# GuidoManni/BodySLAM

Hardware: AMD Instinct MI355X
Metric: frames/sec depth+pose+back-proj, 640x480 seq (higher is better)
Workload: dtype f16

## Files before the change

### bodyslam_amd/_lib.py

```python
from __future__ import annotations

import ctypes as C
import os
from typing import Optional

import torch

_HERE = os.path.dirname(os.path.abspath(__file__))
LIB_PATH = os.environ.get("BODYSLAM_HIP_LIB") or os.path.join(_HERE, "libbodyslam_hip.so")

F32, F16, BF16 = 0, 1, 2
ACT_NONE, ACT_RELU, ACT_GELU, ACT_SOFTPLUS, ACT_SOFTPLUS_FAST = 0, 1, 2, 3, 4
OUT_PLAIN, OUT_SHUFFLE, OUT_QKV = 0, 1, 2

_TORCH2BS = {torch.float32: F32, torch.float16: F16, torch.bfloat16: BF16}
BS2TORCH = {F32: torch.float32, F16: torch.float16, BF16: torch.bfloat16}


class BodySlamHipError(RuntimeError):
    pass


class GemmDesc(C.Structure):
    _fields_ = [
# ... 71 lines not shown
    "bs_odo_p2p_step": [C.c_void_p, C.c_void_p, C.c_int32, C.c_int32, C.c_int32, C.c_void_p, C.c_void_p, C.c_int32, C.c_double, C.c_double, C.c_void_p,
                        C.c_void_p, C.c_void_p],
    "bs_tsdf_touch": [C.c_void_p, C.c_int32, C.c_int32, C.c_int32, C.c_void_p, C.c_void_p, C.c_double, C.c_double, C.c_void_p, C.c_void_p, C.c_void_p,
                      C.c_int32, C.c_int32, C.c_void_p, C.c_int32, C.c_void_p, C.c_void_p, C.c_void_p],
    "bs_tsdf_integrate": [C.c_void_p, C.c_void_p, C.c_int32, C.c_int32, C.c_void_p, C.c_void_p, C.c_void_p, C.c_void_p, C.c_int32, C.c_void_p, C.c_int32,
                          C.c_int32, C.c_double, C.c_double, C.c_void_p, C.c_void_p],
    "bs_tsdf_extract": [C.c_void_p, C.c_int32, C.c_void_p, C.c_void_p, C.c_int32, C.c_void_p, C.c_int32, C.c_int32, C.c_double, C.c_void_p, C.c_void_p,
                        C.c_void_p, C.c_void_p, C.c_void_p, C.c_void_p],
    "bs_tsdf_mesh": [C.c_void_p, C.c_int32, C.c_void_p, C.c_void_p, C.c_int32, C.c_void_p, C.c_int32, C.c_int32, C.c_double, C.c_void_p, C.c_int32] + [C.c_void_p] * 7,
    "bs_tsdf_raycast": [C.c_void_p, C.c_void_p, C.c_int32, C.c_int32, C.c_int32, C.c_double, C.c_double, C.c_void_p, C.c_void_p, C.c_int32, C.c_void_p,
                        C.c_int32, C.c_int32, C.c_double, C.c_double, C.c_void_p, C.c_void_p, C.c_void_p, C.c_void_p, C.c_void_p],
    "bs_attractor_step": [C.c_void_p] * 4 + [C.c_int32] * 8 + [C.c_void_p],
    "bs_add_resized": [C.c_void_p] * 3 + [C.c_int32] * 7 + [C.c_void_p],
    "bs_mlp2": [C.c_void_p, C.c_int32] + [C.c_void_p] * 5 + [C.c_int32] * 6 + [C.c_void_p],
    "bs_mlp2_add": [C.c_void_p] * 7 + [C.c_int32] * 10 + [C.c_void_p],
    "bs_projector_level": [C.c_void_p] * 10 + [C.c_int32] * 9 + [C.c_void_p],
    "bs_logbinom_depth": [C.c_void_p] * 8 + [C.c_int32] * 5 + [C.c_float, C.c_float, C.c_int32, C.c_void_p],
    "bs_logbinom_depth_ex": [C.c_void_p] * 7 + [C.c_int32] + [C.c_void_p] * 2 + [C.c_int32] * 5 + [C.c_float, C.c_float, C.c_int32, C.c_void_p],
    "bs_small_attention": [C.c_void_p, C.c_void_p, C.c_int32, C.c_int32, C.c_int32, C.c_int32, C.c_void_p],
    "bs_route_argmax": [C.c_void_p, C.c_int32, C.c_void_p, C.c_int32, C.c_void_p],
    "bs_postprocess_depth": [C.c_void_p] * 3 + [C.c_int32] * 6 + [C.c_void_p],
    "bs_cyclepose_im2col": [C.c_void_p] * 3 + [C.c_int32] * 4 + [C.c_void_p],
    "bs_cyclepose_im2col_window": [C.c_void_p] * 3 + [C.c_int32] * 8 + [C.c_void_p],
    "bs_instnorm_relu_nhwc": [C.c_void_p] * 4 + [C.c_int32] * 3 + [C.c_float, C.c_int32, C.c_void_p],
    "bs_avgpool_nhwc": [C.c_void_p, C.c_void_p, C.c_int32, C.c_int32, C.c_int32, C.c_void_p],
    "bs_cyclepose_head": [C.c_void_p] * 12 + [C.c_int32] * 3 + [C.c_void_p],
    "bs_backproject": [C.c_void_p, C.c_int32, C.c_int32, C.c_int32, C.c_void_p, C.c_double, C.c_double] + [C.c_void_p] * 6,
    "bs_pose_chain": [C.c_void_p, C.c_int32, C.c_void_p, C.c_void_p, C.c_void_p],
    "bs_pose_chain_from": [C.c_void_p, C.c_int32, C.c_void_p, C.c_void_p, C.c_void_p],
    "bs_pixel_to_3d": [C.c_void_p, C.c_int64, C.c_void_p, C.c_void_p, C.c_void_p],
# ... 426 lines not shown

def resize_bias_relu_nhwc(x, bias, out, B, Hin, Win, Cch, Hout, Wout, split=False):
    check(load_library().bs_resize_bias_relu_nhwc(p(x), p(bias), p(out), B, Hin, Win, Cch, Hout, Wout, 1 | (2 if split else 0), dt(out), stream_ptr()),
          "bs_resize_bias_relu_nhwc")


def attractor_step(A, bins_prev, bins_out, route, B, Hp, Wp, H, W, groups, n_bins, n_attr):
    check(load_library().bs_attractor_step(p(A), p(bins_prev), p(bins_out), p(route), B, Hp, Wp, H, W, groups, n_bins, n_attr,
                                           stream_ptr()), "bs_attractor_step")


def mlp2(x, ldx, W1, b1, W2, b2, out, M, K1, N1, N2, act2=ACT_SOFTPLUS_FAST):
    check(load_library().bs_mlp2(p(x), ldx, p(W1), p(b1), p(W2), p(b2), p(out), M, K1, N1, N2, act2, dt(x), stream_ptr()), "bs_mlp2")


def mlp2_add(emb, prev, W1, b1, W2, b2, out, B, Hp, Wp, H, W, K1, N1, N2, act2=ACT_SOFTPLUS_FAST, split=False):
    check(load_library().bs_mlp2_add(p(emb), p(prev), p(W1), p(b1), p(W2), p(b2), p(out), B, Hp, Wp, H, W, K1, N1, N2, act2,
                                     dt(emb) | (16 if split else 0), stream_ptr()), "bs_mlp2_add")


def projector_level(z, b_c1, emb_prev, Wc2, b_c2, We, b_e, x_out, emb_out, eh_out, B, Hl, Wl, H, W, PM, E, NE):
    check(load_library().bs_projector_level(p(z), p(b_c1), p(emb_prev), p(Wc2), p(b_c2), p(We), p(b_e), p(x_out), p(emb_out), p(eh_out), B, Hl, Wl,
                                            H, W, PM, E, NE, dt(z), stream_ptr()), "bs_projector_level")


def add_resized(x, prev, out, B, Hp, Wp, H, W, Cch, split=False):
    check(load_library().bs_add_resized(p(x), p(prev), p(out), B, Hp, Wp, H, W, Cch, dt(x) | (16 if split else 0), stream_ptr()),
          "bs_add_resized")


# ... 74 lines not shown
```

### bodyslam_amd/csrc/common.h

```cpp
#pragma once
#include <hip/hip_runtime.h>
#include <stdint.h>
#include <stdio.h>
#include <stdlib.h>

#include <atomic>

#include "../../include/bodyslam_hip.h"

namespace bs {

typedef _Float16 f16;
typedef __bf16 bf16;
typedef _Float16 f16x4 __attribute__((ext_vector_type(4)));
typedef _Float16 f16x8 __attribute__((ext_vector_type(8)));
typedef __bf16 bf16x4 __attribute__((ext_vector_type(4)));
typedef __bf16 bf16x8 __attribute__((ext_vector_type(8)));
typedef float f32x4 __attribute__((ext_vector_type(4)));
typedef float f32x16 __attribute__((ext_vector_type(16)));
typedef unsigned int u32x4 __attribute__((ext_vector_type(4)));
typedef unsigned int u32x2 __attribute__((ext_vector_type(2)));

void set_error(const char* fmt, ...);
const void* zero_page();
// ... 138 lines not shown

__device__ __forceinline__ int f8_pack4(float a, float b, float c, float d) {
    auto cl = [](float v) { return __builtin_amdgcn_fmed3f(v, -448.0f, 448.0f); };
    int r = 0;
    r = __builtin_amdgcn_cvt_pk_fp8_f32(cl(a), cl(b), r, false);
    r = __builtin_amdgcn_cvt_pk_fp8_f32(cl(c), cl(d), r, true);
    return r;
}
__device__ __forceinline__ void f8_unpack4(int packed, float (&o)[4]) {
    typedef float f32x2 __attribute__((ext_vector_type(2)));
    const f32x2 a = __builtin_amdgcn_cvt_pk_f32_fp8(packed, false), b = __builtin_amdgcn_cvt_pk_f32_fp8(packed, true);
    o[0] = a[0]; o[1] = a[1]; o[2] = b[0]; o[3] = b[1];
}
constexpr int F8_ACT_HI_EXP = BS_F8_ACT_HI_EXP, F8_ACT_LO_EXP = BS_F8_ACT_LO_EXP;

__device__ __forceinline__ void glds16(const void* gptr, void* lds_wave_base) {
    __builtin_amdgcn_global_load_lds((const __attribute__((address_space(1))) void*)gptr,
                                     (__attribute__((address_space(3))) void*)lds_wave_base, 16, 0, 0);
}

static inline int cdiv(int a, int b) { return (a + b - 1) / b; }
static inline int64_t cdiv64(int64_t a, int64_t b) { return (a + b - 1) / b; }

}
```

### bodyslam_amd/csrc/engine.hip

```cpp
#include <stdio.h>
#include <string.h>

#include <exception>
#include <map>
#include <string>
#include <tuple>
#include <type_traits>
#include <utility>
#include <memory>
#include <vector>

#include "common.h"

namespace {

constexpr char kMagic[8] = {'B', 'S', 'E', 'N', 'G', '0', '2', '\0'};
enum { KIND_WORKSPACE = 0, KIND_ZERO = 1, KIND_DATA = 2 };
enum { ARG_I64 = 0, ARG_F64 = 1, ARG_PTR = 2, ARG_NULL = 3, ARG_DESC = 4 };
enum { OP_CALL = 0, OP_SIGNAL = 1, OP_WAIT = 2 };

struct Arg {
    int64_t i = 0;
    double d = 0.0;
    void* p = nullptr;
// ... 28 lines not shown
}
#define BS_ENGINE_ENTRY(name) {#name, make_entry(name)}
const std::map<std::string, Entry>& entries() {
    static const std::map<std::string, Entry> m = {
        BS_ENGINE_ENTRY(bs_gemm),           BS_ENGINE_ENTRY(bs_attention),          BS_ENGINE_ENTRY(bs_attention_table),
        BS_ENGINE_ENTRY(bs_attention_table_corr),
        BS_ENGINE_ENTRY(bs_layernorm),      BS_ENGINE_ENTRY(bs_cast),               BS_ENGINE_ENTRY(bs_copy_f32),
        BS_ENGINE_ENTRY(bs_cast_split),     BS_ENGINE_ENTRY(bs_relu_split),         BS_ENGINE_ENTRY(bs_preprocess_patches),
        BS_ENGINE_ENTRY(bs_fill_rows),      BS_ENGINE_ENTRY(bs_upconv_tapsum),      BS_ENGINE_ENTRY(bs_small_attention),
        BS_ENGINE_ENTRY(bs_route_argmax),   BS_ENGINE_ENTRY(bs_resize_bilinear_nhwc), BS_ENGINE_ENTRY(bs_rank1_bias),
        BS_ENGINE_ENTRY(bs_postprocess_depth), BS_ENGINE_ENTRY(bs_logbinom_depth_ex), BS_ENGINE_ENTRY(bs_col_mean),
        BS_ENGINE_ENTRY(bs_attractor_step), BS_ENGINE_ENTRY(bs_add_resized),        BS_ENGINE_ENTRY(bs_instnorm_relu_nhwc),
        BS_ENGINE_ENTRY(bs_cyclepose_im2col), BS_ENGINE_ENTRY(bs_cyclepose_im2col_window), BS_ENGINE_ENTRY(bs_cyclepose_head),
        BS_ENGINE_ENTRY(bs_avgpool_nhwc),   BS_ENGINE_ENTRY(bs_mlp2),            BS_ENGINE_ENTRY(bs_mlp2_add),
        BS_ENGINE_ENTRY(bs_upconv_fused),   BS_ENGINE_ENTRY(bs_resize_bias_relu_nhwc), BS_ENGINE_ENTRY(bs_projector_level),
    };
    return m;
}

struct Op {
    int kind = OP_CALL, lane = 0;
    const Entry* entry = nullptr;
    std::vector<Arg> args;
    std::vector<char> desc;
    std::string name;
};
struct Io {
    void* ptr;
    int64_t nbytes;
};
// ... 313 lines not shown
```

### bodyslam_amd/csrc/metric.hip

```cpp
#include "common.h"

namespace bs {

struct Lerp2 {
    int y0, y1, x0, x1;
    float ly, lx, hy, hx;
};
__device__ __forceinline__ Lerp2 lerp_ac(int oy, int ox, int Hin, int Win, float sy, float sx) {
    Lerp2 l;
    const float fy = sy * (float)oy, fx = sx * (float)ox;
    l.y0 = (int)fy;
    l.x0 = (int)fx;
    l.y0 = l.y0 > Hin - 1 ? Hin - 1 : l.y0;
    l.x0 = l.x0 > Win - 1 ? Win - 1 : l.x0;
    l.y1 = l.y0 + (l.y0 < Hin - 1 ? 1 : 0);
    l.x1 = l.x0 + (l.x0 < Win - 1 ? 1 : 0);
    l.ly = fy - (float)l.y0;
    l.lx = fx - (float)l.x0;
    l.hy = 1.0f - l.ly;
    l.hx = 1.0f - l.lx;
    return l;
}

template <int NQ>
__global__ __launch_bounds__(256) void attractor_kernel(const float* A, const float* bins_prev, float* bins_out, const int32_t* route,
                                                         int B, int Hp, int Wp, int H, int W, int G, int nb, int na, float sy, float sx) {
    const int q4 = nb / (4 * NQ);
    const int GG = route ? 1 : G;
    const unsigned per_row = (unsigned)W * GG * q4;
    const unsigned idx = blockIdx.x * blockDim.x + threadIdx.x;
    if (idx >= per_row) return;
    const int b = blockIdx.y / H, oy = blockIdx.y - b * H;
    const int q = idx % q4;
    const int g = route ? route[b] : (int)((idx / q4) % G);
    const int ox = idx / (q4 * GG);
    const int64_t pix = ((int64_t)b * H + oy) * W + ox;
    const Lerp2 l = lerp_ac(oy, ox, Hp, Wp, sy, sx);
// ... 474 lines not shown
```

### bodyslam_amd/csrc/mlp2.hip

```cpp
#include "common.h"

namespace bs {

constexpr int MLP_BM = 256, MLP_K1 = 128, MLP_N1 = 256, MLP_LDS = 131072;

struct MlpAddGeom {
    const void* prev;
    int Hp, Wp, H, W;
    float sy, sx;
};

template <typename T, int FUSE, int SPLIT>
__global__ __launch_bounds__(512) void mlp2_kernel(const T* __restrict__ x, int ldx, const T* __restrict__ W1, const float* __restrict__ b1,
                                                   const T* __restrict__ W2, const float* __restrict__ b2, float* __restrict__ out, int M, int N2,
                                                   int act2, MlpAddGeom ag) {
    typedef typename T16<T>::v8 v8;
    typedef typename T16<T>::v4 v4;
    extern __shared__ __attribute__((aligned(16))) char smem[];
    const int tid = threadIdx.x, lane = tid & 63;
    const int wave = __builtin_amdgcn_readfirstlane(tid >> 6);
    const int m0 = blockIdx.x * MLP_BM;
    const int frow = lane & 15, fq = lane >> 4;

    {
// ... 173 lines not shown
    hipLaunchKernelGGL((mlp2_kernel<T, FUSE, SPLIT>), dim3(cdiv(M, MLP_BM)), dim3(512), MLP_LDS + (FUSE ? MLP_BM * 32 : 0), st, (const T*)x, ldx, (const T*)W1, b1, (const T*)W2, b2,
                       out, M, N2, act2, ag);
    BS_CHECK_LAUNCH();
    return BS_OK;
}

static int mlp2_check(const char* who, const void* x, const void* W1, const float* b1, const void* W2, const float* b2, float* out, int M, int K1,
                      int N1, int N2, int act2, int dtype) {
    if (!initialized()) { set_error("%s: call bs_init first", who); return BS_ERR_NOT_INIT; }
    BS_REQUIRE(x && W1 && b1 && W2 && b2 && out, "%s: null operand", who);
    BS_REQUIRE(dtype == BS_F16 || dtype == BS_BF16, "%s: dtype must be f16 or bf16", who);
    BS_REQUIRE(K1 == MLP_K1 && N1 == MLP_N1, "%s: built for K1 = %d, N1 = %d (got %d, %d)", who, MLP_K1, MLP_N1, K1, N1);
    BS_REQUIRE(N2 > 0 && N2 <= 32 && N2 % 4 == 0, "%s: N2 = %d must be a multiple of 4 in 4 .. 32", who, N2);
    BS_REQUIRE(M > 0, "%s: M = %d", who, M);
    BS_REQUIRE(act2 == BS_ACT_NONE || act2 == BS_ACT_RELU || act2 == BS_ACT_SOFTPLUS || act2 == BS_ACT_SOFTPLUS_FAST || act2 == BS_ACT_GELU, "%s: unknown activation %d", who, act2);
    return BS_OK;
}

}

extern "C" int bs_mlp2(const void* x, int32_t ldx, const void* W1, const float* b1, const void* W2, const float* b2, float* out, int32_t M,
                       int32_t K1, int32_t N1, int32_t N2, int32_t act2, int32_t dtype, void* stream) {
    using namespace bs;
    const int rc = mlp2_check("bs_mlp2", x, W1, b1, W2, b2, out, M, K1, N1, N2, act2, dtype);
    if (rc != BS_OK) return rc;
    BS_REQUIRE(ldx >= K1 && ldx % 8 == 0, "bs_mlp2: ldx = %d (rows of >= K1 16-bit values, 16-byte aligned)", ldx);
    hipStream_t st = (hipStream_t)stream;
    const MlpAddGeom ag{};
    return dtype == BS_F16 ? launch_mlp2<f16, 0, 0>(x, ldx, W1, b1, W2, b2, out, M, N2, act2, ag, st)
                           : launch_mlp2<bf16, 0, 0>(x, ldx, W1, b1, W2, b2, out, M, N2, act2, ag, st);
// ... 11 lines not shown
    if (rc != BS_OK) return rc;
    BS_REQUIRE(prev, "bs_mlp2_add: null operand");
    BS_REQUIRE((int64_t)B * Hp * Wp * K1 * (split ? 2 : 1) < 0x7FFFFFFFll, "bs_mlp2_add: prev too large for 32-bit element offsets");
    MlpAddGeom ag;
    ag.prev = prev; ag.Hp = Hp; ag.Wp = Wp; ag.H = H; ag.W = W;
    ag.sy = H > 1 ? (float)(Hp - 1) / (float)(H - 1) : 0.f;
    ag.sx = W > 1 ? (float)(Wp - 1) / (float)(W - 1) : 0.f;
    const int ldx = K1 * (split ? 2 : 1);
    hipStream_t st = (hipStream_t)stream;
    if (dtype == BS_F16)
        return split ? launch_mlp2<f16, 1, 1>(emb, ldx, W1, b1, W2, b2, out, M, N2, act2, ag, st)
                     : launch_mlp2<f16, 1, 0>(emb, ldx, W1, b1, W2, b2, out, M, N2, act2, ag, st);
    return split ? launch_mlp2<bf16, 1, 1>(emb, ldx, W1, b1, W2, b2, out, M, N2, act2, ag, st)
                 : launch_mlp2<bf16, 1, 0>(emb, ldx, W1, b1, W2, b2, out, M, N2, act2, ag, st);
}
```

### bodyslam_amd/zoedepth.py

```python
from __future__ import annotations

import math
import os
import warnings
import dataclasses
from dataclasses import dataclass
from typing import Dict, Optional, Sequence, Tuple

import numpy as np
import torch
import torch.nn.functional as F

from . import _lib as L
from .calibration import DEFAULT_POLICY, NECK_RELHEAD_WONLY, CalibrationPolicy, Scope, choose, finish_report, saving_gflop, worst

LOG2E = 1.4426950408889634


@dataclass
class ZoeConfig:
    hidden: int = 1024
    layers: int = 24
    heads: int = 16
    intermediate: int = 4096
# ... 625 lines not shown
        else:
            blk = torch.empty((nbytes + 255) // 256 * 256, dtype=torch.uint8, device=self.dev)
            self.bytes_new += blk.numel()
            self.blocks.append(blk)
        t = blk[:nbytes].view(dtype).view(*shape)
        self.owner[t.data_ptr()] = blk
        return t

    def free(self, *tensors):
        for t in tensors:
            blk = self.owner.pop(t.data_ptr(), None) if t is not None else None
            if blk is not None:
                self.free_blocks.append(blk)


class _ZoePlan:

    MEAN_STEP = 8
    F8O = (L.F8_ACT_HI_EXP, L.F8_ACT_LO_EXP)

    def __init__(self, eng: ZoeDepthEngine, B: int, H: int, W: int, flip: bool):
        self.eng, self.c, self.w = eng, eng.cfg, eng.w
        c = eng.cfg
        self.B, self.H, self.W, self.flip = B, H, W, flip
        self.NB = NB = 2 * B if flip else B
        self.nh, self.nw = nh_, nw_ = net_size(H, W, eng.target_hw)
        self.hp, self.wp = hp, wp = nh_ // c.patch, nw_ // c.patch
        self.T0 = T0 = hp * wp
        self.S = S = T0 + 1
        self.Sp = Sp = (S + 63) // 64 * 64
# ... 381 lines not shown
            self.nplain("rh.conv2", r1, "rh.conv2.w", y9, NB * h3 * w3, 9 * c.rel_features, Fc // 2, out_pairs=False, tile=2)
            free(r1)
            last = e16(NB, 2 * h3, 2 * w3, c.rel_features * m2)
            P.add("rh.tapsum", "bs_upconv_tapsum", y9, w["rh.conv2.b"], last, NB, h3, w3, c.rel_features, 2 * h3, 2 * w3, self.RZ, 1, L.dt(last))
            free(y9)
        P.mark("rel_features", last, ("nhwc", NB, 2 * h3, 2 * w3, c.rel_features, self.mfmt()))
        return last

    def _projector_level_fits(self, fused_list, pj_low):
        c, w, eng = self.c, self.w, self.eng
        return (os.environ.get("BS_PROJECTOR_LEVEL", "1") != "0" and self.acc and c.proj_mlp == 64 and c.bin_dim == 128
                and 2 * c.clb_hidden <= 80 and (2 * c.clb_hidden) % 16 == 0 and eng.fuse_mlp
                and all(fw_ % 32 == 0 and 2 * zw_ == fw_ and 2 * zh_ == fh_ for (_, fh_, fw_), (_, zh_, zw_) in zip(fused_list, pj_low))
                and all(tuple(w[f"at{i_}.c1.w"].shape) == (256, 128) and 2 * eng.na_eff[i_] <= 32 for i_ in range(4)))

    def _attractor_step(self, i, A, bins_prev, ph_, pw_, fh, fw):
        NB, nb = self.NB, self.c.n_bins
        bins = self.e32(NB, fh, fw, 2 * nb)
        self.plan.add(f"at{i}.step", "bs_attractor_step", A, bins_prev, bins, self.route, NB, ph_, pw_, fh, fw, 2, nb, self.eng.na_eff[i])
        self.pool.free(A, bins_prev)
        self.plan.mark(f"bins{i}", bins, ("nhwc_route", NB, fh, fw, 2 * nb))
        return bins

    def _levels_fused(self, fused_list, pj_low, bins_prev, emb_prev, ph_, pw_):
        c, w, P, eng, NB, m2 = self.c, self.w, self.plan, self.eng, self.NB, self.m2
        e16, e32, free = self.e16, self.e32, self.pool.free
        E, PM, HID = c.bin_dim, c.proj_mlp, c.clb_hidden
        Eh = None
        for i in range(4):
            _, fh, fw = fused_list[i]
            Mi = NB * fh * fw
            z, zh, zw = pj_low[i]
            assert (zh, zw) == (ph_, pw_), "the projector's low-resolution map and the previous level's embedding share a grid"
            last_lv = i == 3
            x16 = e16(Mi, E)
            emb = None if last_lv else e16(Mi, E * m2)
            if last_lv:
                Eh = e32(Mi, 2 * HID)
            P.add(f"pj{i}.level", "bs_projector_level", z, w[f"pj{i}.c1.b"], emb_prev, w[f"pj{i}.c2.w"], w[f"pj{i}.c2.b"],
                  w["clb.e1.w"] if last_lv else None, w["clb.e1.b"] if last_lv else None, x16, emb, Eh, NB, zh, zw, fh, fw, PM, E, 2 * HID,
                  L.dt(x16))
            f_alg = 2.0 * Mi * PM * (E + (2 * HID if last_lv else 0))
            P.tag_stack(f_alg, 3.0 * f_alg)
            free(z, emb_prev)
            na = eng.na_eff[i]
            A = e32(Mi, 2 * na)
            P.add(f"at{i}.mlp", "bs_mlp2", x16, E, w[f"at{i}.c1.w"], w[f"at{i}.c1.b"], w[f"at{i}.c2.w"], w[f"at{i}.c2.b"], A, Mi, E, 2 * E,
                  2 * na, L.ACT_SOFTPLUS_FAST, L.dt(x16))
            P.tag_stack(2.0 * Mi * (E * 2 * E + 2 * E * 2 * na), 2.0 * Mi * (E * 2 * E + 2 * E * 2 * na))
            free(x16)
            bins_prev = self._attractor_step(i, A, bins_prev, ph_, pw_, fh, fw)
            emb_prev, ph_, pw_ = emb, fh, fw
        return bins_prev, Eh, ph_, pw_

    def _levels_four(self, fused_list, pj_low, bins_prev, emb_prev, ph_, pw_):
        c, w, P, eng, NB, acc, m2, np3 = self.c, self.w, self.plan, self.eng, self.NB, self.acc, self.m2, self.np3
        e16, e32, free = self.e16, self.e32, self.pool.free
        E, PM, HID = c.bin_dim, c.proj_mlp, c.clb_hidden
        for i in range(4):
            _, fh, fw = fused_list[i]
            Mi = NB * fh * fw
            e1 = e16(Mi, PM * m2)
            z, zh, zw = pj_low[i]
            P.add(f"pj{i}.up", "bs_resize_bias_relu_nhwc", z, w[f"pj{i}.c1.b"], e1, NB, zh, zw, PM, fh, fw, 1 | (2 if acc else 0), L.dt(e1))
            free(z)
            emb = e16(Mi, E * m2)
            P.gemm(f"pj{i}.c2", e1, w[f"pj{i}.c2.w"], emb, M=Mi, N=E, K=PM * np3, lda=PM * m2, seg1=PM if acc else 0,
                   ldo=E * m2, out_split_off=E if acc else 0, bias=w[f"pj{i}.c2.b"], precision_passes=np3)
            if i < 3:
                free(e1)
            na = eng.na_eff[i]
            A = e32(Mi, 2 * na)
            fuse = E == 128 and 2 * na <= 32 and eng.fuse_mlp and tuple(w[f"at{i}.c1.w"].shape) == (256, 128)
            f_mlp = 2.0 * Mi * (E * 2 * E + 2 * E * 2 * na)
            if fuse and eng.fuse_mlp > 1:
                P.add(f"at{i}.mlp", "bs_mlp2_add", emb, emb_prev, w[f"at{i}.c1.w"], w[f"at{i}.c1.b"], w[f"at{i}.c2.w"], w[f"at{i}.c2.b"], A, NB, ph_,
                      pw_, fh, fw, E, 2 * E, 2 * na, L.ACT_SOFTPLUS_FAST, L.dt(emb) | (16 if acc else 0))
                P.tag_stack(f_mlp, f_mlp)
                free(emb_prev)
            else:
                y = e16(Mi, E * m2)
                P.add(f"at{i}.add", "bs_add_resized", emb, emb_prev, y, NB, ph_, pw_, fh, fw, E, L.dt(y) | (16 if acc else 0))
                free(emb_prev)
                if fuse:
                    P.add(f"at{i}.mlp", "bs_mlp2", y, E * m2, w[f"at{i}.c1.w"], w[f"at{i}.c1.b"], w[f"at{i}.c2.w"], w[f"at{i}.c2.b"], A, Mi, E, 2 * E,
                          2 * na, L.ACT_SOFTPLUS_FAST, L.dt(y))
# ... 33 lines not shown
```

### include/bodyslam_hip.h

```cpp
#ifndef BODYSLAM_HIP_H
#define BODYSLAM_HIP_H

#include <stdint.h>

#ifdef __cplusplus
extern "C" {
#endif

typedef enum {
    BS_OK = 0,
    BS_ERR_INVALID = -1,
    BS_ERR_HIP = -2,
    BS_ERR_NOT_INIT = -3
} bs_status;

enum { BS_F32 = 0, BS_F16 = 1, BS_BF16 = 2 };
enum { BS_ACT_NONE = 0, BS_ACT_RELU = 1, BS_ACT_GELU = 2, BS_ACT_SOFTPLUS = 3, BS_ACT_SOFTPLUS_FAST = 4 };
enum { BS_OUT_PLAIN = 0, BS_OUT_SHUFFLE = 1, BS_OUT_QKV = 2 };

int bs_init(int device);
const char* bs_last_error(void);
int bs_version(void);

#define BS_F8_ACT_HI_EXP 0
// ... 87 lines not shown
int bs_upconv_tapsum(const float* y, const float* bias, void* out, int32_t B, int32_t Hin, int32_t Win, int32_t Cout,
                     int32_t Hout, int32_t Wout, int32_t align_corners, int32_t relu, int32_t dtype, void* stream);

int bs_upconv_fused(const void* x, const void* w, const float* bias, void* out, int32_t B, int32_t Hin, int32_t Win, int32_t Cin,
                    int32_t Cout, int32_t Hout, int32_t Wout, int32_t flags, int32_t relu, int32_t mode, int32_t sa0, int32_t sb0,
                    int32_t sa1, int32_t sb1, int32_t dtype, void* stream);

int bs_attractor_step(const float* A, const float* bins_prev, float* bins_out, const int32_t* route, int32_t B,
                      int32_t Hp, int32_t Wp, int32_t H, int32_t W, int32_t groups, int32_t n_bins, int32_t n_attr,
                      void* stream);
int bs_mlp2(const void* x, int32_t ldx, const void* W1, const float* b1, const void* W2, const float* b2, float* out, int32_t M,
            int32_t K1, int32_t N1, int32_t N2, int32_t act2, int32_t dtype, void* stream);
int bs_mlp2_add(const void* emb, const void* prev, const void* W1, const float* b1, const void* W2, const float* b2, float* out,
                int32_t B, int32_t Hp, int32_t Wp, int32_t H, int32_t W, int32_t K1, int32_t N1, int32_t N2, int32_t act2, int32_t dtype,
                void* stream);
int bs_projector_level(const void* z, const float* b_c1, const void* emb_prev, const void* Wc2, const float* b_c2, const void* We,
                       const float* b_e, void* x_out, void* emb_out, float* eh_out, int32_t B, int32_t Hl, int32_t Wl, int32_t H, int32_t W,
                       int32_t PM, int32_t E, int32_t NE, int32_t dtype, void* stream);
int bs_add_resized(const void* x, const void* prev, void* out, int32_t B, int32_t Hp, int32_t Wp, int32_t H,
                   int32_t W, int32_t C, int32_t dtype, void* stream);
int bs_logbinom_depth(const void* last, const float* Eh, const float* bins, const float* w0_last, const float* w2,
                      const float* b2, const int32_t* route, float* depth, int32_t B, int32_t H, int32_t W,
                      int32_t He, int32_t We, float min_temp, float max_temp, int32_t dtype, void* stream);
int bs_logbinom_depth_ex(const void* last, const float* Eh, const float* bins, const float* w0_last, const float* w2,
                         const float* b2, const float* rel_w, int32_t hid, const int32_t* route, float* depth, int32_t B,
                         int32_t H, int32_t W, int32_t He, int32_t We, float min_temp, float max_temp, int32_t dtype,
                         void* stream);
int bs_small_attention(const float* qkv, void* out, int32_t B, int32_t S, int32_t nheads, int32_t dtype, void* stream);
int bs_route_argmax(const float* logits, int32_t ld, int32_t* route, int32_t B, void* stream);

// ... 96 lines not shown
```

Measured before the change: 490.0.

## Fuse attractor MLP and bin update into one routed level kernel

Adds a kernel that runs the attractor MLP (two GEMMs via MFMA) for only the routed expert group and then applies the attractor bin update in the same launch. It also bilinearly upsamples the previous bins and, in the add variant, the previous embedding in-kernel. This replaces the separate mlp2 or mlp2_add launch plus attractor_step launch and removes the round trip of the intermediate attractor tensor through global memory. Work is restricted to the routed group instead of both. It adds a large LDS footprint, which limits occupancy, and it only applies when n_bins is 64 and the effective attractor count is at most 16.

Result: no change. 493.8, median of 6 (+0.8%).

```diff
diff --git a/bodyslam_amd/_lib.py b/bodyslam_amd/_lib.py
--- a/bodyslam_amd/_lib.py
+++ b/bodyslam_amd/_lib.py
@@ -109,6 +109,8 @@
     "bs_add_resized": [C.c_void_p] * 3 + [C.c_int32] * 7 + [C.c_void_p],
     "bs_mlp2": [C.c_void_p, C.c_int32] + [C.c_void_p] * 5 + [C.c_int32] * 6 + [C.c_void_p],
     "bs_mlp2_add": [C.c_void_p] * 7 + [C.c_int32] * 10 + [C.c_void_p],
+    "bs_attractor_level": [C.c_void_p, C.c_int32] + [C.c_void_p] * 7 + [C.c_int32] * 11 + [C.c_void_p],
+    "bs_attractor_level_add": [C.c_void_p] * 9 + [C.c_int32] * 11 + [C.c_void_p],
     "bs_projector_level": [C.c_void_p] * 10 + [C.c_int32] * 9 + [C.c_void_p],
     "bs_logbinom_depth": [C.c_void_p] * 8 + [C.c_int32] * 5 + [C.c_float, C.c_float, C.c_int32, C.c_void_p],
     "bs_logbinom_depth_ex": [C.c_void_p] * 7 + [C.c_int32] + [C.c_void_p] * 2 + [C.c_int32] * 5 + [C.c_float, C.c_float, C.c_int32, C.c_void_p],
@@ -565,6 +567,18 @@
     check(load_library().bs_mlp2(p(x), ldx, p(W1), p(b1), p(W2), p(b2), p(out), M, K1, N1, N2, act2, dt(x), stream_ptr()), "bs_mlp2")
 
 
+def attractor_level(x, ldx, W1, b1, W2, b2, bins_prev, bins_out, route, B, Hp, Wp, H, W, K1, N1, n_bins, n_attr, act2=ACT_SOFTPLUS_FAST):
+    check(load_library().bs_attractor_level(p(x), ldx, p(W1), p(b1), p(W2), p(b2), p(bins_prev), p(bins_out), p(route), B, Hp, Wp, H, W, K1, N1,
+                                            n_bins, n_attr, act2, dt(x), stream_ptr()), "bs_attractor_level")
+
+
+def attractor_level_add(emb, prev, W1, b1, W2, b2, bins_prev, bins_out, route, B, Hp, Wp, H, W, K1, N1, n_bins, n_attr, act2=ACT_SOFTPLUS_FAST,
+                        split=False):
+    check(load_library().bs_attractor_level_add(p(emb), p(prev), p(W1), p(b1), p(W2), p(b2), p(bins_prev), p(bins_out), p(route), B, Hp, Wp, H, W,
+                                                K1, N1, n_bins, n_attr, act2, dt(emb) | (16 if split else 0), stream_ptr()),
+          "bs_attractor_level_add")
+
+
 def mlp2_add(emb, prev, W1, b1, W2, b2, out, B, Hp, Wp, H, W, K1, N1, N2, act2=ACT_SOFTPLUS_FAST, split=False):
     check(load_library().bs_mlp2_add(p(emb), p(prev), p(W1), p(b1), p(W2), p(b2), p(out), B, Hp, Wp, H, W, K1, N1, N2, act2,
                                      dt(emb) | (16 if split else 0), stream_ptr()), "bs_mlp2_add")
diff --git a/bodyslam_amd/csrc/common.h b/bodyslam_amd/csrc/common.h
--- a/bodyslam_amd/csrc/common.h
+++ b/bodyslam_amd/csrc/common.h
@@ -176,6 +176,26 @@
 }
 constexpr int F8_ACT_HI_EXP = BS_F8_ACT_HI_EXP, F8_ACT_LO_EXP = BS_F8_ACT_LO_EXP;
 
+struct Lerp2 {
+    int y0, y1, x0, x1;
+    float ly, lx, hy, hx;
+};
+__device__ __forceinline__ Lerp2 lerp_ac(int oy, int ox, int Hin, int Win, float sy, float sx) {
+    Lerp2 l;
+    const float fy = sy * (float)oy, fx = sx * (float)ox;
+    l.y0 = (int)fy;
+    l.x0 = (int)fx;
+    l.y0 = l.y0 > Hin - 1 ? Hin - 1 : l.y0;
+    l.x0 = l.x0 > Win - 1 ? Win - 1 : l.x0;
+    l.y1 = l.y0 + (l.y0 < Hin - 1 ? 1 : 0);
+    l.x1 = l.x0 + (l.x0 < Win - 1 ? 1 : 0);
+    l.ly = fy - (float)l.y0;
+    l.lx = fx - (float)l.x0;
+    l.hy = 1.0f - l.ly;
+    l.hx = 1.0f - l.lx;
+    return l;
+}
+
 __device__ __forceinline__ void glds16(const void* gptr, void* lds_wave_base) {
     __builtin_amdgcn_global_load_lds((const __attribute__((address_space(1))) void*)gptr,
                                      (__attribute__((address_space(3))) void*)lds_wave_base, 16, 0, 0);
diff --git a/bodyslam_amd/csrc/engine.hip b/bodyslam_amd/csrc/engine.hip
--- a/bodyslam_amd/csrc/engine.hip
+++ b/bodyslam_amd/csrc/engine.hip
@@ -66,6 +66,7 @@
         BS_ENGINE_ENTRY(bs_cyclepose_im2col), BS_ENGINE_ENTRY(bs_cyclepose_im2col_window), BS_ENGINE_ENTRY(bs_cyclepose_head),
         BS_ENGINE_ENTRY(bs_avgpool_nhwc),   BS_ENGINE_ENTRY(bs_mlp2),            BS_ENGINE_ENTRY(bs_mlp2_add),
         BS_ENGINE_ENTRY(bs_upconv_fused),   BS_ENGINE_ENTRY(bs_resize_bias_relu_nhwc), BS_ENGINE_ENTRY(bs_projector_level),
+        BS_ENGINE_ENTRY(bs_attractor_level), BS_ENGINE_ENTRY(bs_attractor_level_add),
     };
     return m;
 }
diff --git a/bodyslam_amd/csrc/metric.hip b/bodyslam_amd/csrc/metric.hip
--- a/bodyslam_amd/csrc/metric.hip
+++ b/bodyslam_amd/csrc/metric.hip
@@ -1,26 +1,6 @@
 #include "common.h"
 
 namespace bs {
-
-struct Lerp2 {
-    int y0, y1, x0, x1;
-    float ly, lx, hy, hx;
-};
-__device__ __forceinline__ Lerp2 lerp_ac(int oy, int ox, int Hin, int Win, float sy, float sx) {
-    Lerp2 l;
-    const float fy = sy * (float)oy, fx = sx * (float)ox;
-    l.y0 = (int)fy;
-    l.x0 = (int)fx;
-    l.y0 = l.y0 > Hin - 1 ? Hin - 1 : l.y0;
-    l.x0 = l.x0 > Win - 1 ? Win - 1 : l.x0;
-    l.y1 = l.y0 + (l.y0 < Hin - 1 ? 1 : 0);
-    l.x1 = l.x0 + (l.x0 < Win - 1 ? 1 : 0);
-    l.ly = fy - (float)l.y0;
-    l.lx = fx - (float)l.x0;
-    l.hy = 1.0f - l.ly;
-    l.hx = 1.0f - l.lx;
-    return l;
-}
 
 template <int NQ>
 __global__ __launch_bounds__(256) void attractor_kernel(const float* A, const float* bins_prev, float* bins_out, const int32_t* route,
diff --git a/bodyslam_amd/csrc/mlp2.hip b/bodyslam_amd/csrc/mlp2.hip
--- a/bodyslam_amd/csrc/mlp2.hip
+++ b/bodyslam_amd/csrc/mlp2.hip
@@ -211,6 +211,270 @@
     BS_REQUIRE(N2 > 0 && N2 <= 32 && N2 % 4 == 0, "%s: N2 = %d must be a multiple of 4 in 4 .. 32", who, N2);
     BS_REQUIRE(M > 0, "%s: M = %d", who, M);
     BS_REQUIRE(act2 == BS_ACT_NONE || act2 == BS_ACT_RELU || act2 == BS_ACT_SOFTPLUS || act2 == BS_ACT_SOFTPLUS_FAST || act2 == BS_ACT_GELU, "%s: unknown activation %d", who, act2);
+    return BS_OK;
+}
+
+constexpr int AL_BM = 128, AL_NB = 64, AL_LDS = 32768 + 32768 + AL_BM * 16 * 4;
+
+template <typename T, int FUSE, int SPLIT>
+__global__ __launch_bounds__(256, 2) void attractor_level_kernel(const T* __restrict__ x, int ldx, const T* __restrict__ prev, const T* __restrict__ W1,
+                                                                 const float* __restrict__ b1, const T* __restrict__ W2,
+                                                                 const float* __restrict__ b2, const float* __restrict__ bins_prev,
+                                                                 float* __restrict__ bins_out, const int32_t* __restrict__ route, int Hp, int Wp,
+                                                                 int H, int W, int na, int act2, float sy, float sx) {
+    typedef typename T16<T>::v8 v8;
+    typedef typename T16<T>::v4 v4;
+    extern __shared__ __attribute__((aligned(16))) char smem[];
+    constexpr int XS = 16384;
+    char* const wsm = smem + 2 * XS;
+    float* const atile = reinterpret_cast<float*>(smem + 4 * XS);
+    const int tid = threadIdx.x, lane = tid & 63;
+    const int wave = __builtin_amdgcn_readfirstlane(tid >> 6);
+    const int b = blockIdx.y, hw = H * W, p0 = blockIdx.x * AL_BM;
+    int g = route[b];
+    g = g < 0 ? 0 : (g > 1 ? 1 : g);
+    const int frow = lane & 15, fq = lane >> 4;
+    const int CB = 2 * AL_NB;
+
+    {
+        const int r8 = lane >> 3, chunk = (lane & 7) ^ r8;
+        const T* xb = x + (int64_t)b * hw * ldx;
+        const char* wl = reinterpret_cast<const char*>(W1 + (int64_t)(g * 128 + r8) * MLP_K1 + chunk * 8);
+#pragma unroll
+        for (int it = 0; it < 4; ++it) {
+            const int rg = wave + it * 4;
+            int p = p0 + rg * 8 + r8;
+            p = p < hw ? p : hw - 1;
+            const char* xs = reinterpret_cast<const char*>(xb + (int64_t)p * ldx + chunk * 8);
+#pragma unroll
+            for (int seg = 0; seg < 2; ++seg) {
+                if (!FUSE) glds16(xs + seg * 128, smem + seg * XS + rg * 1024);
+                glds16(wl + (int64_t)rg * 8 * MLP_K1 * 2 + seg * 128, wsm + seg * XS + rg * 1024);
+            }
+        }
+    }
+    const int q = tid & 7;
+    float c[4][8];
+    {
+        const float* pb = bins_prev + (int64_t)b * Hp * Wp * CB + g * AL_NB + q * 8;
+#pragma unroll
+        for (int k0 = 0; k0 < 4; k0 += 2) {
+            f32x4 p00[2][2], p01[2][2], p10[2][2], p11[2][2];
+            Lerp2 l[2];
+#pragma unroll
+            for (int k = 0; k < 2; ++k) {
+                int p = p0 + (tid >> 3) + 32 * (k0 + k);
+                p = p < hw ? p : hw - 1;
+                const int oy = p / W, ox = p - oy * W;
+                l[k] = lerp_ac(oy, ox, Hp, Wp, sy, sx);
+#pragma unroll
+                for (int u = 0; u < 2; ++u) {
+                    p00[k][u] = *reinterpret_cast<const f32x4*>(pb + ((int64_t)l[k].y0 * Wp + l[k].x0) * CB + 4 * u);
+                    p01[k][u] = *reinterpret_cast<const f32x4*>(pb + ((int64_t)l[k].y0 * Wp + l[k].x1) * CB + 4 * u);
+                    p10[k][u] = *reinterpret_cast<const f32x4*>(pb + ((int64_t)l[k].y1 * Wp + l[k].x0) * CB + 4 * u);
+                    p11[k][u] = *reinterpret_cast<const f32x4*>(pb + ((int64_t)l[k].y1 * Wp + l[k].x1) * CB + 4 * u);
+                }
+            }
+#pragma unroll
+            for (int k = 0; k < 2; ++k)
+#pragma unroll
+                for (int u = 0; u < 2; ++u)
+#pragma unroll
+                    for (int e = 0; e < 4; ++e)
+                        c[k0 + k][4 * u + e] = l[k].hy * (l[k].hx * p00[k][u][e] + l[k].lx * p01[k][u][e]) + l[k].ly * (l[k].hx * p10[k][u][e] + l[k].lx * p11[k][u][e]);
+#pragma unroll
+            for (int k = 0; k < 2; ++k)
+#pragma unroll
+                for (int e = 0; e < 8; ++e) asm volatile("" : "+v"(c[k0 + k][e]));
+        }
+    }
+    v8 w2f[4];
+#pragma unroll
+    for (int ks = 0; ks < 4; ++ks) {
+        v8 z;
+#pragma unroll
+        for (int e = 0; e < 8; ++e) z[e] = T16<T>::from_f32(0.f);
+        w2f[ks] = frow < na ? *reinterpret_cast<const v8*>(W2 + (int64_t)(g * na + frow) * MLP_N1 + g * 128 + ks * 32 + fq * 8) : z;
+    }
+    if constexpr (FUSE) {
+        constexpr int C = MLP_K1, PS = SPLIT ? 2 : 1;
+        auto ld8 = [&](const T* ptr, float (&dst)[8]) {
+            const v8 h = *reinterpret_cast<const v8*>(ptr);
+#pragma unroll
+            for (int e = 0; e < 8; ++e) dst[e] = (float)h[e];
+            if (SPLIT) {
+                const v8 l = *reinterpret_cast<const v8*>(ptr + C);
+#pragma unroll
+                for (int e = 0; e < 8; ++e) dst[e] += (float)l[e];
+            }
+        };
+        typedef int i32x4_ __attribute__((ext_vector_type(4)));
+        i32x4_* rtab = reinterpret_cast<i32x4_*>(atile);
+        const T* xb = x + (int64_t)b * hw * ldx;
+        if (tid < AL_BM) {
+            int p = p0 + tid;
+            p = p < hw ? p : hw - 1;
+            const int oy = p / W, ox = p - oy * W;
+            const float fy = sy * (float)oy, fx = sx * (float)ox;
+            int y0 = (int)fy, x0 = (int)fx;
+            y0 = y0 > Hp - 1 ? Hp - 1 : y0;
+            x0 = x0 > Wp - 1 ? Wp - 1 : x0;
+            const int y1 = y0 + (y0 < Hp - 1 ? 1 : 0), x1 = x0 + (x0 < Wp - 1 ? 1 : 0);
+            const float ly = fy - (float)y0, lx = fx - (float)x0, hy = 1.0f - ly, hx = 1.0f - lx;
+            const int pb0 = b * Hp * Wp;
+            rtab[2 * tid] = i32x4_{(pb0 + y0 * Wp + x0) * C * PS, (pb0 + y0 * Wp + x1) * C * PS, (pb0 + y1 * Wp + x0) * C * PS,
+                                   (pb0 + y1 * Wp + x1) * C * PS};
+            rtab[2 * tid + 1] = i32x4_{__float_as_int(hx), __float_as_int(lx), __float_as_int(hy), __float_as_int(ly)};
+        }
+        __syncthreads();
+#pragma unroll 2
+        for (int k = 0; k < AL_BM * 16 / 256; ++k) {
+            const int idx = tid + k * 256, r = idx >> 4, c8 = idx & 15;
+            int p = p0 + r;
+            p = p < hw ? p : hw - 1;
+            const i32x4_ po = rtab[2 * r], pw = rtab[2 * r + 1];
+            const float hx = __int_as_float(pw[0]), lx = __int_as_float(pw[1]), hy = __int_as_float(pw[2]), ly = __int_as_float(pw[3]);
+            const T* pp = prev + c8 * 8;
+            float q00[8], q01[8], q10[8], q11[8], av[8];
+            ld8(pp + po[0], q00);
+            ld8(pp + po[1], q01);
+            ld8(pp + po[2], q10);
+            ld8(pp + po[3], q11);
+            ld8(xb + (int64_t)p * ldx + c8 * 8, av);
+            const f32x2_ hx2 = {hx, hx}, lx2 = {lx, lx}, hy2 = {hy, hy}, ly2 = {ly, ly};
+            v8 o;
+#pragma unroll
+            for (int e = 0; e < 8; e += 2) {
+                f32x2_ v = bilerp2(f32x2_{q00[e], q00[e + 1]}, f32x2_{q01[e], q01[e + 1]}, f32x2_{q10[e], q10[e + 1]}, f32x2_{q11[e], q11[e + 1]}, hx2, lx2,
+                                   hy2, ly2);
+                v += f32x2_{av[e], av[e + 1]};
+                o[e] = T16<T>::from_f32(v[0]);
+                o[e + 1] = T16<T>::from_f32(v[1]);
+            }
+            *reinterpret_cast<v8*>(smem + (c8 >> 3) * XS + r * 128 + (((c8 & 7) ^ (r & 7)) << 4)) = o;
+        }
+    }
+    asm volatile("s_waitcnt vmcnt(0)" ::: "memory");
+    __syncthreads();
+
+    const int wr = wave >> 1, wc = wave & 1;
+    f32x4 acc1[4][4];
+#pragma unroll
+    for (int i = 0; i < 4; ++i)
+#pragma unroll
+        for (int j = 0; j < 4; ++j) acc1[i][j] = f32x4{0.f, 0.f, 0.f, 0.f};
+    const int sw = frow & 7;
+#pragma unroll
+    for (int ks = 0; ks < 4; ++ks) {
+        const int seg = ks >> 1, kc = (ks & 1) * 4;
+        const int coff = ((kc + fq) ^ sw) << 4;
+        v8 xf[4], wf[4];
+#pragma unroll
+        for (int i = 0; i < 4; ++i) xf[i] = *reinterpret_cast<const v8*>(smem + seg * XS + (wr * 64 + i * 16 + frow) * 128 + coff);
+#pragma unroll
+        for (int j = 0; j < 4; ++j) wf[j] = *reinterpret_cast<const v8*>(wsm + seg * XS + (wc * 64 + j * 16 + frow) * 128 + coff);
+#pragma unroll
+        for (int i = 0; i < 4; ++i)
+#pragma unroll
+            for (int j = 0; j < 4; ++j) acc1[i][j] = T16<T>::mfma16(wf[j], xf[i], acc1[i][j]);
+    }
+    __syncthreads();
+#pragma unroll
+    for (int j = 0; j < 4; ++j) {
+        const int n = wc * 64 + j * 16 + fq * 4;
+        const f32x4 bb = *reinterpret_cast<const f32x4*>(b1 + g * 128 + n);
+        const int seg = n >> 6, chunk = (n & 63) >> 3, sub = (n & 7) * 2;
+#pragma unroll
+        for (int i = 0; i < 4; ++i) {
+            const int m = wr * 64 + i * 16 + frow;
+            v4 h;
+#pragma unroll
+            for (int e = 0; e < 4; ++e) h[e] = T16<T>::from_f32(fmaxf(acc1[i][j][e] + bb[e], 0.0f));
+            *reinterpret_cast<v4*>(smem + seg * XS + m * 128 + ((chunk ^ (m & 7)) << 4) + sub) = h;
+        }
+    }
+    __syncthreads();
+
+    f32x4 acc2[2];
+#pragma unroll
+    for (int i = 0; i < 2; ++i) acc2[i] = f32x4{0.f, 0.f, 0.f, 0.f};
+#pragma unroll
+    for (int ks = 0; ks < 4; ++ks) {
+        const int seg = ks >> 1, kc = (ks & 1) * 4;
+        const int coff = ((kc + fq) ^ sw) << 4;
+#pragma unroll
+        for (int i = 0; i < 2; ++i) {
+            const v8 af = *reinterpret_cast<const v8*>(smem + seg * XS + (wave * 32 + i * 16 + frow) * 128 + coff);
+            acc2[i] = T16<T>::mfma16(w2f[ks], af, acc2[i]);
+        }
+    }
+    if (fq * 4 < na) {
+        const f32x4 bb = *reinterpret_cast<const f32x4*>(b2 + g * na + fq * 4);
+#pragma unroll 1
+        for (int i = 0; i < 2; ++i) {
+            f32x4 y;
+#pragma unroll
+            for (int e = 0; e < 4; ++e) y[e] = apply_act(acc2[i][e] + bb[e], act2);
+            *reinterpret_cast<f32x4*>(atile + (wave * 32 + i * 16 + frow) * 16 + fq * 4) = y;
+        }
+    }
+    __syncthreads();
+
+#pragma unroll
+    for (int k = 0; k < 4; ++k) {
+        const int pl = (tid >> 3) + 32 * k;
+        float dsum[8];
+#pragma unroll
+        for (int e = 0; e < 8; ++e) dsum[e] = 0.f;
+        for (int a4 = 0; a4 < na; a4 += 4) {
+            const f32x4 av = *reinterpret_cast<const f32x4*>(atile + pl * 16 + a4);
+#pragma unroll
+            for (int kk = 0; kk < 4; ++kk)
+#pragma unroll
+                for (int h = 0; h < 4; ++h) {
+                    const f32x2_ dx = f32x2_{av[kk], av[kk]} - f32x2_{c[k][2 * h], c[k][2 * h + 1]};
+                    const f32x2_ den = __builtin_elementwise_fma(dx * f32x2_{300.0f, 300.0f}, dx, f32x2_{1.0f, 1.0f});
+                    const f32x2_ r = {__builtin_amdgcn_rcpf(den[0]), __builtin_amdgcn_rcpf(den[1])};
+                    const f32x2_ d2 = __builtin_elementwise_fma(dx, r, f32x2_{dsum[2 * h], dsum[2 * h + 1]});
+                    dsum[2 * h] = d2[0];
+                    dsum[2 * h + 1] = d2[1];
+                }
+        }
+        const int p = p0 + pl;
+        if (p < hw) {
+            float* po = bins_out + ((int64_t)b * hw + p) * CB + g * AL_NB + q * 8;
+#pragma unroll
+            for (int u = 0; u < 2; ++u) {
+                f32x4 o;
+#pragma unroll
+                for (int e = 0; e < 4; ++e) o[e] = c[k][4 * u + e] + dsum[4 * u + e] / (float)na;
+                *reinterpret_cast<f32x4*>(po + 4 * u) = o;
+            }
+        }
+    }
+}
+
+template <typename T, int FUSE, int SPLIT>
+static int launch_attractor_level(const void* x, int ldx, const void* prev, const void* W1, const float* b1, const void* W2, const float* b2,
+                                  const float* bins_prev, float* bins_out, const int32_t* route, int B, int Hp, int Wp, int H, int W, int na, int act2,
+                                  hipStream_t st) {
+    BS_MAX_DYNAMIC_LDS(((const void*)attractor_level_kernel<T, FUSE, SPLIT>), AL_LDS);
+    const float sy = H > 1 ? (float)(Hp - 1) / (float)(H - 1) : 0.f, sx = W > 1 ? (float)(Wp - 1) / (float)(W - 1) : 0.f;
+    hipLaunchKernelGGL((attractor_level_kernel<T, FUSE, SPLIT>), dim3(cdiv(H * W, AL_BM), B), dim3(256), AL_LDS, st, (const T*)x, ldx, (const T*)prev,
+                       (const T*)W1, b1, (const T*)W2, b2, bins_prev, bins_out, route, Hp, Wp, H, W, na, act2, sy, sx);
+    BS_CHECK_LAUNCH();
+    return BS_OK;
+}
+
+static int attractor_level_check(const char* who, const void* x, const void* W1, const float* b1, const void* W2, const float* b2,
+                                 const float* bins_prev, float* bins_out, const int32_t* route, int B, int Hp, int Wp, int H, int W, int K1, int N1,
+                                 int n_bins, int n_attr, int act2, int dtype) {
+    BS_REQUIRE(B > 0 && B <= 65535 && Hp > 0 && Wp > 0 && H > 0 && W > 0 && (int64_t)B * H * W < 0x7FFFFFFFll, "%s: bad geometry", who);
+    BS_REQUIRE(n_attr > 0 && n_attr <= 16 && n_attr % 4 == 0, "%s: n_attr = %d must be a multiple of 4 in 4 .. 16", who, n_attr);
+    const int rc = mlp2_check(who, x, W1, b1, W2, b2, bins_out, B * H * W, K1, N1, 2 * n_attr, act2, dtype);
+    if (rc != BS_OK) return rc;
+    BS_REQUIRE(bins_prev && route, "%s: null operand (bins_prev and route are required)", who);
+    BS_REQUIRE(n_bins == AL_NB, "%s: built for n_bins = %d (got %d)", who, AL_NB, n_bins);
     return BS_OK;
 }
 
@@ -252,3 +516,37 @@
     return split ? launch_mlp2<bf16, 1, 1>(emb, ldx, W1, b1, W2, b2, out, M, N2, act2, ag, st)
                  : launch_mlp2<bf16, 1, 0>(emb, ldx, W1, b1, W2, b2, out, M, N2, act2, ag, st);
 }
+
+extern "C" int bs_attractor_level(const void* x, int32_t ldx, const void* W1, const float* b1, const void* W2, const float* b2,
+                                  const float* bins_prev, float* bins_out, const int32_t* route, int32_t B, int32_t Hp, int32_t Wp, int32_t H,
+                                  int32_t W, int32_t K1, int32_t N1, int32_t n_bins, int32_t n_attr, int32_t act2, int32_t dtype, void* stream) {
+    using namespace bs;
+    const int rc = attractor_level_check("bs_attractor_level", x, W1, b1, W2, b2, bins_prev, bins_out, route, B, Hp, Wp, H, W, K1, N1, n_bins, n_attr,
+                                         act2, dtype);
+    if (rc != BS_OK) return rc;
+    BS_REQUIRE(ldx >= K1 && ldx % 8 == 0, "bs_attractor_level: ldx = %d (rows of >= K1 16-bit values, 16-byte aligned)", ldx);
+    hipStream_t st = (hipStream_t)stream;
+    return dtype == BS_F16
+               ? launch_attractor_level<f16, 0, 0>(x, ldx, nullptr, W1, b1, W2, b2, bins_prev, bins_out, route, B, Hp, Wp, H, W, n_attr, act2, st)
+               : launch_attractor_level<bf16, 0, 0>(x, ldx, nullptr, W1, b1, W2, b2, bins_prev, bins_out, route, B, Hp, Wp, H, W, n_attr, act2, st);
+}
+
+extern "C" int bs_attractor_level_add(const void* emb, const void* prev, const void* W1, const float* b1, const void* W2, const float* b2,
+                                      const float* bins_prev, float* bins_out, const int32_t* route, int32_t B, int32_t Hp, int32_t Wp, int32_t H,
+                                      int32_t W, int32_t K1, int32_t N1, int32_t n_bins, int32_t n_attr, int32_t act2, int32_t dtype,
+                                      void* stream) {
+    using namespace bs;
+    const int split = (dtype & 16) ? 1 : 0;
+    dtype &= 15;
+    const int rc = attractor_level_check("bs_attractor_level_add", emb, W1, b1, W2, b2, bins_prev, bins_out, route, B, Hp, Wp, H, W, K1, N1, n_bins,
+                                         n_attr, act2, dtype);
+    if (rc != BS_OK) return rc;
+    BS_REQUIRE(prev, "bs_attractor_level_add: null operand");
+    BS_REQUIRE((int64_t)B * Hp * Wp * K1 * (split ? 2 : 1) < 0x7FFFFFFFll, "bs_attractor_level_add: prev too large for 32-bit element offsets");
+    const int ldx = K1 * (split ? 2 : 1);
+    hipStream_t st = (hipStream_t)stream;
+#define BS_AL_ADD(T, S) launch_attractor_level<T, 1, S>(emb, ldx, prev, W1, b1, W2, b2, bins_prev, bins_out, route, B, Hp, Wp, H, W, n_attr, act2, st)
+    if (dtype == BS_F16) return split ? BS_AL_ADD(f16, 1) : BS_AL_ADD(f16, 0);
+    return split ? BS_AL_ADD(bf16, 1) : BS_AL_ADD(bf16, 0);
+#undef BS_AL_ADD
+}
diff --git a/bodyslam_amd/zoedepth.py b/bodyslam_amd/zoedepth.py
--- a/bodyslam_amd/zoedepth.py
+++ b/bodyslam_amd/zoedepth.py
@@ -1,5 +1,6 @@
 from __future__ import annotations
 
+import contextlib
 import math
 import os
 import warnings
@@ -663,6 +664,15 @@
                 self.free_blocks.append(blk)
 
 
+@contextlib.contextmanager
+def two_launch_attractor():
+    _ZoePlan.routed_level = False
+    try:
+        yield
+    finally:
+        _ZoePlan.routed_level = True
+
+
 class _ZoePlan:
 
     MEAN_STEP = 8
@@ -1074,6 +1084,29 @@
                 and all(fw_ % 32 == 0 and 2 * zw_ == fw_ and 2 * zh_ == fh_ for (_, fh_, fw_), (_, zh_, zw_) in zip(fused_list, pj_low))
                 and all(tuple(w[f"at{i_}.c1.w"].shape) == (256, 128) and 2 * eng.na_eff[i_] <= 32 for i_ in range(4)))
 
+    routed_level = True
+
+    def _routed_level_fits(self, i):
+        c, eng = self.c, self.eng
+        return (self.routed_level and c.bin_dim == 128 and c.n_bins == 64 and eng.na_eff[i] <= 16 and eng.fuse_mlp
+                and tuple(self.w[f"at{i}.c1.w"].shape) == (256, 128))
+
+    def _attractor_level(self, i, x, ldx, prev, bins_prev, ph_, pw_, fh, fw):
+        c, w, P, NB = self.c, self.w, self.plan, self.NB
+        E, nb, na, Mi = c.bin_dim, c.n_bins, self.eng.na_eff[i], self.NB * fh * fw
+        bins = self.e32(NB, fh, fw, 2 * nb)
+        wts = (w[f"at{i}.c1.w"], w[f"at{i}.c1.b"], w[f"at{i}.c2.w"], w[f"at{i}.c2.b"])
+        tail = (bins_prev, bins, self.route, NB, ph_, pw_, fh, fw, E, 2 * E, nb, na, L.ACT_SOFTPLUS_FAST)
+        if prev is None:
+            P.add(f"at{i}.level", "bs_attractor_level", x, ldx, *wts, *tail, L.dt(x))
+        else:
+            P.add(f"at{i}.level", "bs_attractor_level_add", x, prev, *wts, *tail, L.dt(x) | (16 if self.acc else 0))
+        f_lv = 2.0 * Mi * (E * E + E * na)
+        P.tag_stack(f_lv, f_lv)
+        self.pool.free(bins_prev)
+        P.mark(f"bins{i}", bins, ("nhwc_route", NB, fh, fw, 2 * nb))
+        return bins
+
     def _attractor_step(self, i, A, bins_prev, ph_, pw_, fh, fw):
         NB, nb = self.NB, self.c.n_bins
         bins = self.e32(NB, fh, fw, 2 * nb)
@@ -1104,6 +1137,11 @@
             P.tag_stack(f_alg, 3.0 * f_alg)
             free(z, emb_prev)
             na = eng.na_eff[i]
+            if self._routed_level_fits(i):
+                bins_prev = self._attractor_level(i, x16, E, None, bins_prev, ph_, pw_, fh, fw)
+                free(x16)
+                emb_prev, ph_, pw_ = emb, fh, fw
+                continue
             A = e32(Mi, 2 * na)
             P.add(f"at{i}.mlp", "bs_mlp2", x16, E, w[f"at{i}.c1.w"], w[f"at{i}.c1.b"], w[f"at{i}.c2.w"], w[f"at{i}.c2.b"], A, Mi, E, 2 * E,
                   2 * na, L.ACT_SOFTPLUS_FAST, L.dt(x16))
@@ -1130,6 +1168,11 @@
             if i < 3:
                 free(e1)
             na = eng.na_eff[i]
+            if eng.fuse_mlp > 1 and self._routed_level_fits(i):
+                bins_prev = self._attractor_level(i, emb, None, emb_prev, bins_prev, ph_, pw_, fh, fw)
+                free(emb_prev)
+                emb_prev, ph_, pw_ = emb, fh, fw
+                continue
             A = e32(Mi, 2 * na)
             fuse = E == 128 and 2 * na <= 32 and eng.fuse_mlp and tuple(w[f"at{i}.c1.w"].shape) == (256, 128)
             f_mlp = 2.0 * Mi * (E * 2 * E + 2 * E * 2 * na)
diff --git a/include/bodyslam_hip.h b/include/bodyslam_hip.h
--- a/include/bodyslam_hip.h
+++ b/include/bodyslam_hip.h
@@ -125,6 +125,12 @@
 int bs_mlp2_add(const void* emb, const void* prev, const void* W1, const float* b1, const void* W2, const float* b2, float* out,
                 int32_t B, int32_t Hp, int32_t Wp, int32_t H, int32_t W, int32_t K1, int32_t N1, int32_t N2, int32_t act2, int32_t dtype,
                 void* stream);
+int bs_attractor_level(const void* x, int32_t ldx, const void* W1, const float* b1, const void* W2, const float* b2,
+                       const float* bins_prev, float* bins_out, const int32_t* route, int32_t B, int32_t Hp, int32_t Wp, int32_t H,
+                       int32_t W, int32_t K1, int32_t N1, int32_t n_bins, int32_t n_attr, int32_t act2, int32_t dtype, void* stream);
+int bs_attractor_level_add(const void* emb, const void* prev, const void* W1, const float* b1, const void* W2, const float* b2,
+                           const float* bins_prev, float* bins_out, const int32_t* route, int32_t B, int32_t Hp, int32_t Wp, int32_t H,
+                           int32_t W, int32_t K1, int32_t N1, int32_t n_bins, int32_t n_attr, int32_t act2, int32_t dtype, void* stream);
 int bs_projector_level(const void* z, const float* b_c1, const void* emb_prev, const void* Wc2, const float* b_c2, const void* We,
                        const float* b_e, void* x_out, void* emb_out, float* eh_out, int32_t B, int32_t Hl, int32_t Wl, int32_t H, int32_t W,
                        int32_t PM, int32_t E, int32_t NE, int32_t dtype, void* stream);
```
